# nianticlabs/implicit-depth

Measured on AMD Instinct MI355X. Metric: frames/sec (BDModel.forward hot path, 512x384, 64 planes, 8-frame tuple = 1 current + 7 source views; third-party backbones excluded), higher is better.
Workload: dtype f32

## Files before the change

implicit-depth_amd/_lib.py:

```python
from __future__ import annotations

import ctypes as C
import os

import torch

_HERE = os.path.dirname(os.path.abspath(__file__))
LIB_PATH = os.environ.get("IDH_LIB") or os.path.join(_HERE, "lib", "libidh.so")

_lib = None
MIN_ABI_VERSION = 111

f32p = C.c_void_p


class IdhError(RuntimeError):
    pass


class VolumeOpts(C.Structure):

    _fields_ = [("cur_batch_stride", C.c_int64), ("src_batch_stride", C.c_int64), ("planes", C.c_void_p),
                ("planes_batch_stride", C.c_int64), ("planes_plane_stride", C.c_int64), ("planes_pixel_stride", C.c_int32),
                ("kernel", C.c_int32), ("scratch", C.c_void_p), ("scratch_floats", C.c_int64), ("struct_size", C.c_int64)]

    def __init__(self, *a, **k):
        super().__init__(*a, **k)
        self.struct_size = C.sizeof(VolumeOpts)


CV_KERNEL_LANE, CV_KERNEL_QUAD, CV_KERNEL_WINDOW = 1, 2, 3


class EvalArgs(C.Structure):

    _fields_ = [("struct_size", C.c_int64), ("prediction", C.c_void_p), ("pred_kind", C.c_int32), ("sampling", C.c_int32),
                ("sigmoid_multiplier", C.c_float), ("surface_threshold", C.c_float), ("rendered_bphw", C.c_void_p), ("depth_b1hw", C.c_void_p),
                ("gt_b1HW", C.c_void_p), ("thresholds", C.c_void_p), ("bins", C.c_void_p), ("T", C.c_int32), ("n_bins", C.c_int32),
                ("tag_mask", C.c_int32), ("B", C.c_int32), ("P", C.c_int32), ("h", C.c_int32), ("w", C.c_int32), ("H", C.c_int32), ("W", C.c_int32)]
# ... 471 lines not shown
```

implicit-depth_amd/cost_volume.py:

```python
from __future__ import annotations

from typing import Optional

import torch
from torch import Tensor, nn

from . import _lib
from .geometry import BackprojectDepth, Project3D


def to_nhwc(x_nchw: Tensor) -> Tensor:
    _lib.require_cuda_f32(x_nchw)
    x = x_nchw.contiguous()
    *lead, C, H, W = x.shape
    n_img = 1
    for s in lead:
        n_img *= s
    out = torch.empty(*lead, H, W, C, device=x.device, dtype=torch.float32)
    if out.numel():
        _lib.check(_lib.lib().idh_nchw_to_nhwc_f32(_lib.ptr(x), _lib.ptr(out), n_img, C, H * W, _lib.stream_ptr()), "idh_nchw_to_nhwc_f32")
    return out


def to_nchw(x_nhwc: Tensor) -> Tensor:
# ... 2 lines not shown
    *lead, H, W, C = x.shape
    n_img = 1
    for s in lead:
        n_img *= s
    out = torch.empty(*lead, C, H, W, device=x.device, dtype=torch.float32)
    if out.numel():
        _lib.check(_lib.lib().idh_nhwc_to_nchw_f32(_lib.ptr(x), _lib.ptr(out), n_img, C, H * W, _lib.stream_ptr()), "idh_nhwc_to_nchw_f32")
    return out


def _is_device_scalar(v) -> bool:
    return torch.is_tensor(v) and v.is_cuda


def volume_opts(B, K, C, H, W, D, planes_bdhw: Optional[Tensor] = None, cur_batch_stride: int = 0, src_batch_stride: int = 0, kernel: int = 0,
                dot_scratch_device=None):
    n_scratch = int(_lib.lib().idh_cost_volume_dot_scratch_floats(B, K, C, H, W, D)) if dot_scratch_device is not None else 0
    if planes_bdhw is None and not cur_batch_stride and not src_batch_stride and not kernel and not n_scratch:
        return None, []
    o = _lib.VolumeOpts()
    o.cur_batch_stride, o.src_batch_stride, o.kernel = int(cur_batch_stride), int(src_batch_stride), int(kernel)
    keep = []
    if n_scratch:
        sc = torch.empty(n_scratch, device=dot_scratch_device, dtype=torch.float32)
        o.scratch, o.scratch_floats = sc.data_ptr(), n_scratch
        keep.append(sc)
    if planes_bdhw is not None:
        pl = planes_bdhw
        _lib.require_cuda_f32(pl)
        if pl.dim() != 4 or pl.shape[1] != D or pl.shape[0] not in (1, B) or tuple(pl.shape[2:]) not in ((H, W), (1, 1)):
            raise ValueError(f"depth_planes_bdhw has shape {tuple(pl.shape)}, expected ({B},{D},{H},{W})")
        const_over_image = tuple(pl.shape[2:]) == (1, 1) or (pl.stride(2) == 0 and pl.stride(3) == 0)
        if const_over_image:
            sb = pl.stride(0) if pl.shape[0] == B and B > 1 else 0
            o.planes, o.planes_batch_stride, o.planes_plane_stride, o.planes_pixel_stride = pl.data_ptr(), sb, pl.stride(1), 0
        else:
# ... 160 lines not shown
DEFAULT_MLP_MATH = "fp32"


class FeatureVolumeManager(CostVolumeManager):

    def __init__(self, matching_height, matching_width, num_depth_bins=64, mlp_channels=None, matching_dim_size=16, num_source_views=7):
        super().__init__(matching_height, matching_width, num_depth_bins)
        from .networks import MLP

        mlp_channels = list(mlp_channels) if mlp_channels is not None else [202, 128, 128, 1]
        mlp_channels[0] = matching_dim_size * (1 + num_source_views) + 10 * num_source_views + 4
        self.matching_dim_size = matching_dim_size
        self.num_source_views = num_source_views
        self.mlp = MLP(channel_list=mlp_channels, disable_final_activation=True)
        self.mlp_math: Optional[str] = None

    def _math(self) -> str:
        m = DEFAULT_MLP_MATH if self.__dict__.get("mlp_math") is None else self.mlp_math
        if m not in MLP_MATH_MODES:
            raise _lib.IdhError(f"unknown MLP math mode {m!r} (expected one of {MLP_MATH_MODES})")
        return m

    def _packed(self):
        lins = [self.mlp.net[0], self.mlp.net[2], self.mlp.net[4]]
        math = self._math()
        key = (math,) + tuple((p.data_ptr(), _lib.param_version(p)) for p in self.mlp.parameters())
        c = self.__dict__.get("_idh_fv")
        if c is not None and c[0] == key:
            return c[1]
        K, C = self.num_source_views, self.matching_dim_size
# ... 41 lines not shown
             planes_t=None, cur_batch_stride=0, src_batch_stride=0, scratch=None):
        B, K, C, H, W = dims
        if K != self.num_source_views:
            raise _lib.IdhError(f"FeatureVolumeManager was built for {self.num_source_views} source views, got {K} (the MLP input width is fixed)")
        pk = self._packed()
        L = _lib.lib()
        D = self.num_depth_bins
        sc = scratch if scratch is not None else {}
        key = ("fv", B, H, W, D, str(dev), torch.cuda.current_stream().cuda_stream)
        if sc.get("fv_key") != key:
            wsb = L.idh_feature_volume_workspace_bytes(B)
            sc.update(fv_key=key, fv_wsb=wsb, fv_ws=torch.empty(max(wsb // 4, 1), device=dev), fv_planes=torch.empty(D, device=dev))
        lowest = torch.empty(B, H, W, device=dev)
        mask = torch.empty(B, H, W, device=dev, dtype=torch.bool) if want_mask else None
        planes = sc["fv_planes"] if planes_t is None else None
        opts, keep = volume_opts(B, K, C, H, W, D, planes_t, cur_batch_stride, src_batch_stride)
        mats = [t if t.is_contiguous() else t.contiguous() for t in (src_Ks, src_extrinsics, src_poses, cur_invK)]
        _lib.check(
            L.idh_feature_volume_ex_fwd(cur_ptr, src_ptr, mats[0].data_ptr(), mats[1].data_ptr(), mats[2].data_ptr(), mats[3].data_ptr(),
                                        dmin, dmax, B, K, C, H, W, D,
                                        pk["w1v"].data_ptr(), pk["w1p"].data_ptr(), pk["pose"].data_ptr(), pk["b1"].data_ptr(), pk["w2"].data_ptr(),
                                        pk["vecs"].data_ptr(), vol_ptr, vol_cs, lowest.data_ptr(),
                                        _lib.ptr(mask), _lib.ptr(planes), sc["fv_ws"].data_ptr(), sc["fv_wsb"], int(pk["math"] == "f16x3"), opts,
                                        _lib.stream_ptr()),
            "idh_feature_volume_ex_fwd")
        del keep
        return lowest, planes, mask

    def build_cost_volume(self, cur_feats, src_feats, src_extrinsics, src_poses, src_Ks, cur_invK, min_depth, max_depth,
                          depth_planes_bdhw=None, return_mask=False, cur_feats_nhwc=None, src_feats_nhwc=None):
        B, K, C, H, W = self._check(cur_feats, src_feats)
# ... 28 lines not shown
```

implicit-depth_amd/csrc/feature_volume.hip:

```cpp
#include <stdlib.h>

#include "idh_common.h"
#include "split_f16.h"

namespace {

using namespace idh_f16;

constexpr int kC = 16;
constexpr int kHid = 128;
constexpr int kNS = 8;
constexpr int kMaxK = 8;

constexpr int kWsHom = 0, kWsT = 192, kWsInvK = 256, kWsBias = 272;
static_assert(kWsT == 12 * IDH_MAX_SOURCE_VIEWS && kWsInvK == kWsT + 4 * IDH_MAX_SOURCE_VIEWS && kWsBias + kHid <= 400, "workspace layout");
constexpr int kWsStrideReal = 400;

__device__ __forceinline__ float lrelu01(float x) {
#ifdef IDH_ABL_FV2_NOACT
    return x;
#endif
    return __builtin_elementwise_maximum(x, x * 0.01f);
}
__device__ __forceinline__ float lrelu01_sel(float x) { return x >= 0.f ? x : x * 0.01f; }

__device__ __forceinline__ float fv_depth_plane(int i, int D, float dmin, float dmax) {
    float ramp = 0.f;
    if (D > 1) {
        const float step = 1.0f / (float)(D - 1);
        ramp = (i < D / 2) ? step * (float)i : 1.0f - step * (float)(D - 1 - i);
    }
    return expf(logf(dmin) + logf(dmax / dmin) * ramp);
}

__global__ void fv_setup_k(const float *__restrict__ src_K, const float *__restrict__ src_E,
                           const float *__restrict__ src_poses, const float *__restrict__ cur_invK,
                           const float *__restrict__ w1_pose, const float *__restrict__ b1, int K,
                           float *__restrict__ ws) {
    const int b = blockIdx.x, t = threadIdx.x;
    float *o = ws + (size_t)b * kWsStrideReal;
    __shared__ float s_pd[3 * IDH_MAX_SOURCE_VIEWS];
    if (t < K) {
        const float *Km = src_K + (size_t)(b * K + t) * 16, *Em = src_E + (size_t)(b * K + t) * 16;
        const float *iK = cur_invK + (size_t)b * 16, *Pm = src_poses + (size_t)(b * K + t) * 16;
        float P[3][4];
        for (int i = 0; i < 3; ++i)
            for (int j = 0; j < 4; ++j) {
                float s = 0.f;
                for (int m = 0; m < 4; ++m) s = fmaf(Km[i * 4 + m], Em[m * 4 + j], s);
                P[i][j] = s;
            }
        float *h = o + kWsHom + 12 * t;
        for (int i = 0; i < 3; ++i) {
            for (int j = 0; j < 3; ++j) {
                float s = 0.f;
                for (int m = 0; m < 3; ++m) s = fmaf(P[i][m], iK[m * 4 + j], s);
                h[i * 3 + j] = s;
            }
            h[9 + i] = P[i][3];
        }
        o[kWsT + 4 * t + 0] = Pm[3]; o[kWsT + 4 * t + 1] = Pm[7]; o[kWsT + 4 * t + 2] = Pm[11]; o[kWsT + 4 * t + 3] = 0.f;
        const float tr = Pm[0] + Pm[5] + Pm[10];
        const float rm = sqrtf(2.f * (1.f - fminf(3.f, tr) / 3.f));
        const float tm = sqrtf(Pm[3] * Pm[3] + Pm[7] * Pm[7] + Pm[11] * Pm[11]);
        s_pd[t] = sqrtf(tm * tm + rm * rm);
        s_pd[K + t] = rm;
        s_pd[2 * K + t] = tm;
    }
    if (t < 9) o[kWsInvK + t] = cur_invK[(size_t)b * 16 + (t / 3) * 4 + (t % 3)];
    __syncthreads();
    if (t < kHid) {
        float s = b1[t];
        for (int j = 0; j < 3 * K; ++j) s = fmaf(w1_pose[(size_t)t * 3 * K + j], s_pd[j], s);
        o[kWsBias + t] = s;
    }
}

struct FvArgs {
    const float *cur;
    const float *src;
    const float *ws;
    const float *w1v;
    const float *w1p;
    const float *w2;
    const float *vecs;
    float *vol;
    unsigned char *mask;
    int vol_cs;
    int B, K, H, W, D;
    int tiles_per_img;
    int DP, G;
    int J, MB;
    float dmin, dmax;
    long long cur_bs, src_bs;
    const float *planes;
    long long planes_sb, planes_sd;
    int planes_sp;
};

__device__ __forceinline__ float fv_plane(const FvArgs &a, int b, int p, int d) {
    return a.planes ? a.planes[(size_t)b * a.planes_sb + (size_t)d * a.planes_sd + (size_t)p * a.planes_sp]
                    : fv_depth_plane(d, a.D, a.dmin, a.dmax);
}

template <int KT>
__global__ __launch_bounds__(512) void fv_mlp_k(const FvArgs a) {
    extern __shared__ __attribute__((aligned(16))) unsigned char smem_raw[];
    f32x4 *sW1 = reinterpret_cast<f32x4 *>(smem_raw);
    f32x4 *sW2 = sW1 + (a.K + 4) * kNS * 64;
    {
        const f32x4 *g1 = reinterpret_cast<const f32x4 *>(a.w1v);
        const f32x4 *g2 = reinterpret_cast<const f32x4 *>(a.w2);
        const int n1 = (a.K + 4) * kNS * 64, n2 = kNS * kNS * 64;
        for (int i = threadIdx.x; i < n1; i += 512) sW1[i] = g1[i];
        for (int i = threadIdx.x; i < n2; i += 512) sW2[i] = g2[i];
    }
    __syncthreads();
    const float *s_b2 = a.vecs, *s_w3 = a.vecs + kHid;
    const float b3 = a.vecs[2 * kHid];

    const int lane = threadIdx.x & 63;
// ... 285 lines not shown
                    const float qy = fmaf(hm[3], pxf, fmaf(hm[4], pyf, hm[5]));
                    const float qz = fmaf(hm[6], pxf, fmaf(hm[7], pyf, hm[8]));
                    const float cx = fmaf(depth, qx, hm[9]);
                    const float cy = fmaf(depth, qy, hm[10]);
                    const float cz = fmaf(depth, qz, hm[11]);
                    const float z = fmaxf(cz, 1e-5f);
                    float r = __builtin_amdgcn_rcpf(z);
                    r = r * fmaf(-z, r, 2.0f);
                    const float u = cx * r, v = cy * r;
                    any_inb |= (u > 2.f) & (u < Wf - 2.f) & (v > 2.f) & (v < Hf - 2.f);
                    any_front |= z > 0.f;
                }
                if (q == 0 && live) a.mask[(size_t)b * N + p] = (any_front && any_inb) ? 1 : 0;
            }
            P = Pn; cur = curn; wc = wcn;
        }
    }
}

template <int CB>
__global__ __launch_bounds__(512) void fv_mlp_gen_k(const FvArgs a) {
    extern __shared__ __attribute__((aligned(16))) unsigned char smem_raw[];
    f32x4 *sW2 = reinterpret_cast<f32x4 *>(smem_raw);
    {
        const f32x4 *g2 = reinterpret_cast<const f32x4 *>(a.w2);
        for (int i = threadIdx.x; i < kNS * kNS * 64; i += 512) sW2[i] = g2[i];
    }
    __syncthreads();
    const f32x4 *gW1 = reinterpret_cast<const f32x4 *>(a.w1v);
    const float *s_b2 = a.vecs, *s_w3 = a.vecs + kHid;
// ... 619 lines not shown
                               size_t workspace_bytes, void *stream, bool f16x3, const idh_volume_opts *opts) {
    const bool own_planes = opts && opts->planes;
    if (own_planes) { dmin = dmax = 1.f; planes_d = nullptr; }
    if (B < 0 || K <= 0 || H <= 0 || W <= 0 || D <= 0 || !(dmin > 0.f) || !(dmax > 0.f)) return IDH_EINVAL;
    const bool generic = C != kC || K > kMaxK;
    if ((long long)K * H * W * C * 4 >= (1ll << 31)) return IDH_EUNSUPPORTED;
    if ((C != kC && C != 2 * kC) || K > IDH_MAX_SOURCE_VIEWS || D > 4096 || (generic && f16x3)) return IDH_EUNSUPPORTED;
    if (B == 0) return IDH_OK;
    if (!cur_nhwc || !src_nhwc || !src_K_44 || !src_E_44 || !src_poses_44 || !cur_invK_44 || !w1_voxel_packed ||
        !w1_pixel_packed || !w1_pose_rowmajor || !b1 || !w2_packed || !vecs_b2_w3_b3 || !vol)
        return IDH_EINVAL;
    if (vol_nhwc_cs != 0 && vol_nhwc_cs < D) return IDH_EINVAL;
    if (!workspace || workspace_bytes < idh_feature_volume_workspace_bytes(B)) return IDH_EWORKSPACE;
    hipStream_t st = idh_stream(stream);
    float *ws = static_cast<float *>(workspace);
    hipLaunchKernelGGL(fv_setup_k, dim3(B), dim3(128), 0, st, src_K_44, src_E_44, src_poses_44, cur_invK_44,
                       w1_pose_rowmajor, b1, K, ws);
    IDH_CHECK_LAUNCH();

    FvArgs a{};
    a.cur = cur_nhwc; a.src = src_nhwc; a.ws = ws; a.w1v = static_cast<const float *>(w1_voxel_packed); a.w1p = w1_pixel_packed;
    a.w2 = static_cast<const float *>(w2_packed);
    a.vecs = vecs_b2_w3_b3; a.vol = vol; a.mask = mask_bhw; a.vol_cs = vol_nhwc_cs;
    a.B = B; a.K = K; a.H = H; a.W = W; a.D = D; a.dmin = dmin; a.dmax = dmax;
    const int N = H * W;
    a.cur_bs = (long long)N * C; a.src_bs = (long long)K * N * C;
    a.J = K <= kMaxK ? 2 : (K + 3) / 4;
    a.MB = 2 * a.J;
    if (opts) {
        if (opts->cur_batch_stride) a.cur_bs = opts->cur_batch_stride;
        if (opts->src_batch_stride) a.src_bs = opts->src_batch_stride;
        if (a.cur_bs < (long long)N * C || a.src_bs < (long long)K * N * C || (a.cur_bs & 3) || (a.src_bs & 3)) return IDH_EINVAL;
        if (opts->planes) {
            if (opts->planes_pixel_stride != 0 && opts->planes_pixel_stride != 1) return IDH_EINVAL;
            a.planes = opts->planes; a.planes_sb = opts->planes_batch_stride; a.planes_sd = opts->planes_plane_stride;
            a.planes_sp = opts->planes_pixel_stride;
        }
    }
    a.tiles_per_img = (N + 15) / 16;
    fv_plane_groups(B, H, W, D, &a.G, &a.DP);
    const long long pix_tasks = (long long)B * a.tiles_per_img;
    const long long ntasks = pix_tasks * a.G;
    int grid = (int)((ntasks + 7) / 8);
    if (grid > 256) grid = 256;
    static IdhDeviceOnce attr_set;
    if (attr_set.first()) {
        if (hipFuncSetAttribute(reinterpret_cast<const void *>(fv_mlp_k<0>), hipFuncAttributeMaxDynamicSharedMemorySize,
                                160 * 1024) != hipSuccess ||
            hipFuncSetAttribute(reinterpret_cast<const void *>(fv_mlp_gen_k<1>), hipFuncAttributeMaxDynamicSharedMemorySize, 64 * 1024) != hipSuccess ||
            hipFuncSetAttribute(reinterpret_cast<const void *>(fv_mlp_gen_k<2>), hipFuncAttributeMaxDynamicSharedMemorySize, 64 * 1024) != hipSuccess ||
            hipFuncSetAttribute(reinterpret_cast<const void *>(fv_mlp_k<7>), hipFuncAttributeMaxDynamicSharedMemorySize,
                                160 * 1024) != hipSuccess ||
            hipFuncSetAttribute(reinterpret_cast<const void *>(fv_mlp_k<8>), hipFuncAttributeMaxDynamicSharedMemorySize,
                                160 * 1024) != hipSuccess ||
            hipFuncSetAttribute(reinterpret_cast<const void *>(fv_mlp_f16_k<0>), hipFuncAttributeMaxDynamicSharedMemorySize,
                                160 * 1024) != hipSuccess ||
            hipFuncSetAttribute(reinterpret_cast<const void *>(fv_mlp_f16_k<7>), hipFuncAttributeMaxDynamicSharedMemorySize,
                                160 * 1024) != hipSuccess ||
            hipFuncSetAttribute(reinterpret_cast<const void *>(fv_mlp_f16_k<8>), hipFuncAttributeMaxDynamicSharedMemorySize,
                                160 * 1024) != hipSuccess)
            return IDH_ELAUNCH;
        attr_set.mark();
    }
    if (generic) {
        const size_t lds = (size_t)kNS * kNS * 64 * sizeof(f32x4);
        if (C == kC) hipLaunchKernelGGL(fv_mlp_gen_k<1>, dim3(grid), dim3(512), lds, st, a);
        else hipLaunchKernelGGL(fv_mlp_gen_k<2>, dim3(grid), dim3(512), lds, st, a);
    } else if (f16x3) {
        const int nb32 = (K + 5) / 2;
        const size_t lds = ((size_t)nb32 * kNS * 2 * 64 + 4 * kNS * 2 * 64) * 16;
        const float *sw1 = reinterpret_cast<const float *>(static_cast<const char *>(w1_voxel_packed) + (size_t)nb32 * kNS * 2 * 64 * 16);
        const float *sw2 = reinterpret_cast<const float *>(static_cast<const char *>(w2_packed) + (size_t)4 * kNS * 2 * 64 * 16);
        if (K == 7) hipLaunchKernelGGL(fv_mlp_f16_k<7>, dim3(grid), dim3(512), lds, st, a, sw1, sw2);
        else if (K == 8) hipLaunchKernelGGL(fv_mlp_f16_k<8>, dim3(grid), dim3(512), lds, st, a, sw1, sw2);
        else hipLaunchKernelGGL(fv_mlp_f16_k<0>, dim3(grid), dim3(512), lds, st, a, sw1, sw2);
    } else {
        const size_t lds = ((size_t)(K + 4) * kNS * 64 + kNS * kNS * 64) * sizeof(f32x4);
        if (K == 7) hipLaunchKernelGGL(fv_mlp_k<7>, dim3(grid), dim3(512), lds, st, a);
        else if (K == 8) hipLaunchKernelGGL(fv_mlp_k<8>, dim3(grid), dim3(512), lds, st, a);
        else hipLaunchKernelGGL(fv_mlp_k<0>, dim3(grid), dim3(512), lds, st, a);
    }
    IDH_CHECK_LAUNCH();
    if (lowest_bhw) {
        int g2 = idh_cdiv((long long)B * N, vol_nhwc_cs > 0 ? 16 : 256);
        if (g2 > 8192) g2 = 8192;
        hipLaunchKernelGGL(argmax_planes_k, dim3(g2), dim3(256), 0, st, vol, vol_nhwc_cs, B, N, D, dmin, dmax, lowest_bhw,
                           planes_d, a.planes, a.planes_sb, a.planes_sd, a.planes_sp);
        IDH_CHECK_LAUNCH();
    }
    return IDH_OK;
}
```

include/idh.h:

```cpp
#ifndef IDH_H_
#define IDH_H_

#include <stddef.h>
#include <stdint.h>

#ifdef __cplusplus
extern "C" {
#endif
#if defined(__GNUC__) || defined(__clang__)
#pragma GCC visibility push(default)
#endif

#define IDH_OK 0
#define IDH_EINVAL (-1)
#define IDH_EUNSUPPORTED (-2)
#define IDH_ELAUNCH (-3)
#define IDH_EWORKSPACE (-4)

#define IDH_MAX_SOURCE_VIEWS 16

#define IDH_ACT_NONE 0
#define IDH_ACT_LRELU 1
#define IDH_ACT_ELU 2

// ... 2 lines not shown

int idh_nchw_to_nhwc_f32(const float *src_nchw, float *dst_nhwc, int n_img, int C, int HW, void *stream);
int idh_nhwc_to_nchw_f32(const float *src_nhwc, float *dst_nchw, int n_img, int C, int HW, void *stream);

typedef struct idh_volume_opts {
    int64_t cur_batch_stride;
    int64_t src_batch_stride;
    const float *planes;
    int64_t planes_batch_stride;
    int64_t planes_plane_stride;
    int32_t planes_pixel_stride;
    int32_t kernel;
    float *scratch;
    int64_t scratch_floats;
    int64_t struct_size;
} idh_volume_opts;

size_t idh_sizeof_volume_opts(void);

#define IDH_CV_KERNEL_LANE 1
#define IDH_CV_KERNEL_QUAD 2
#define IDH_CV_KERNEL_WINDOW 3

int idh_cost_volume_dot_fwd(const float *cur_nhwc, const float *src_nhwc, const float *src_K_44,
                            const float *src_E_44, const float *cur_invK_44, float dmin, float dmax,
                            int B, int K, int C, int H, int W, int D, float *cost, int cost_nhwc_cs,
                            float *lowest_bhw, float *planes_d, void *stream);
int idh_cost_volume_dot_ex_fwd(const float *cur_nhwc, const float *src_nhwc, const float *src_K_44,
                               const float *src_E_44, const float *cur_invK_44, float dmin, float dmax,
                               int B, int K, int C, int H, int W, int D, float *cost, int cost_nhwc_cs,
// ... 177 lines not shown
```

Before: 690.3.

## Skip MLP work for source views that project outside the image

Adds a sampled visibility estimate in the setup kernel that measures what fraction of source-view projections fall outside the image. A new skip kernel variant computes an active-view mask per plane and runs the layer-1 accumulation only for views with in-bounds taps. It is used when enough views are empty, with both kernels launched and each exiting early depending on the device-side estimate. This aims to cut wasted bilinear gathers and MFMA work on out-of-frustum views, at the cost of an extra launch, divergent loops, and reliance on those views contributing zero features.

```diff
diff --git a/implicit-depth_amd/_lib.py b/implicit-depth_amd/_lib.py
--- a/implicit-depth_amd/_lib.py
+++ b/implicit-depth_amd/_lib.py
@@ -22,7 +22,8 @@
 
     _fields_ = [("cur_batch_stride", C.c_int64), ("src_batch_stride", C.c_int64), ("planes", C.c_void_p),
                 ("planes_batch_stride", C.c_int64), ("planes_plane_stride", C.c_int64), ("planes_pixel_stride", C.c_int32),
-                ("kernel", C.c_int32), ("scratch", C.c_void_p), ("scratch_floats", C.c_int64), ("struct_size", C.c_int64)]
+                ("kernel", C.c_int32), ("scratch", C.c_void_p), ("scratch_floats", C.c_int64), ("struct_size", C.c_int64),
+                ("fv_keep_empty_views", C.c_int32), ("reserved0", C.c_int32)]
 
     def __init__(self, *a, **k):
         super().__init__(*a, **k)
diff --git a/implicit-depth_amd/cost_volume.py b/implicit-depth_amd/cost_volume.py
--- a/implicit-depth_amd/cost_volume.py
+++ b/implicit-depth_amd/cost_volume.py
@@ -40,12 +40,13 @@
 
 
 def volume_opts(B, K, C, H, W, D, planes_bdhw: Optional[Tensor] = None, cur_batch_stride: int = 0, src_batch_stride: int = 0, kernel: int = 0,
-                dot_scratch_device=None):
+                dot_scratch_device=None, fv_keep_empty_views: int = 0):
     n_scratch = int(_lib.lib().idh_cost_volume_dot_scratch_floats(B, K, C, H, W, D)) if dot_scratch_device is not None else 0
-    if planes_bdhw is None and not cur_batch_stride and not src_batch_stride and not kernel and not n_scratch:
+    if planes_bdhw is None and not cur_batch_stride and not src_batch_stride and not kernel and not n_scratch and not fv_keep_empty_views:
         return None, []
     o = _lib.VolumeOpts()
     o.cur_batch_stride, o.src_batch_stride, o.kernel = int(cur_batch_stride), int(src_batch_stride), int(kernel)
+    o.fv_keep_empty_views = int(fv_keep_empty_views)
     keep = []
     if n_scratch:
         sc = torch.empty(n_scratch, device=dot_scratch_device, dtype=torch.float32)
@@ -236,6 +237,7 @@
         self.num_source_views = num_source_views
         self.mlp = MLP(channel_list=mlp_channels, disable_final_activation=True)
         self.mlp_math: Optional[str] = None
+        self.skip_empty_views = True
 
     def _math(self) -> str:
         m = DEFAULT_MLP_MATH if self.__dict__.get("mlp_math") is None else self.mlp_math
@@ -307,7 +309,8 @@
         lowest = torch.empty(B, H, W, device=dev)
         mask = torch.empty(B, H, W, device=dev, dtype=torch.bool) if want_mask else None
         planes = sc["fv_planes"] if planes_t is None else None
-        opts, keep = volume_opts(B, K, C, H, W, D, planes_t, cur_batch_stride, src_batch_stride)
+        opts, keep = volume_opts(B, K, C, H, W, D, planes_t, cur_batch_stride, src_batch_stride,
+                                 fv_keep_empty_views={True: 0, False: 1, "always": 2}[self.__dict__.get("skip_empty_views", True)])
         mats = [t if t.is_contiguous() else t.contiguous() for t in (src_Ks, src_extrinsics, src_poses, cur_invK)]
         _lib.check(
             L.idh_feature_volume_ex_fwd(cur_ptr, src_ptr, mats[0].data_ptr(), mats[1].data_ptr(), mats[2].data_ptr(), mats[3].data_ptr(),
diff --git a/implicit-depth_amd/csrc/feature_volume.hip b/implicit-depth_amd/csrc/feature_volume.hip
--- a/implicit-depth_amd/csrc/feature_volume.hip
+++ b/implicit-depth_amd/csrc/feature_volume.hip
@@ -31,49 +31,6 @@
         ramp = (i < D / 2) ? step * (float)i : 1.0f - step * (float)(D - 1 - i);
     }
     return expf(logf(dmin) + logf(dmax / dmin) * ramp);
-}
-
-__global__ void fv_setup_k(const float *__restrict__ src_K, const float *__restrict__ src_E,
-                           const float *__restrict__ src_poses, const float *__restrict__ cur_invK,
-                           const float *__restrict__ w1_pose, const float *__restrict__ b1, int K,
-                           float *__restrict__ ws) {
-    const int b = blockIdx.x, t = threadIdx.x;
-    float *o = ws + (size_t)b * kWsStrideReal;
-    __shared__ float s_pd[3 * IDH_MAX_SOURCE_VIEWS];
-    if (t < K) {
-        const float *Km = src_K + (size_t)(b * K + t) * 16, *Em = src_E + (size_t)(b * K + t) * 16;
-        const float *iK = cur_invK + (size_t)b * 16, *Pm = src_poses + (size_t)(b * K + t) * 16;
-        float P[3][4];
-        for (int i = 0; i < 3; ++i)
-            for (int j = 0; j < 4; ++j) {
-                float s = 0.f;
-                for (int m = 0; m < 4; ++m) s = fmaf(Km[i * 4 + m], Em[m * 4 + j], s);
-                P[i][j] = s;
-            }
-        float *h = o + kWsHom + 12 * t;
-        for (int i = 0; i < 3; ++i) {
-            for (int j = 0; j < 3; ++j) {
-                float s = 0.f;
-                for (int m = 0; m < 3; ++m) s = fmaf(P[i][m], iK[m * 4 + j], s);
-                h[i * 3 + j] = s;
-            }
-            h[9 + i] = P[i][3];
-        }
-        o[kWsT + 4 * t + 0] = Pm[3]; o[kWsT + 4 * t + 1] = Pm[7]; o[kWsT + 4 * t + 2] = Pm[11]; o[kWsT + 4 * t + 3] = 0.f;
-        const float tr = Pm[0] + Pm[5] + Pm[10];
-        const float rm = sqrtf(2.f * (1.f - fminf(3.f, tr) / 3.f));
-        const float tm = sqrtf(Pm[3] * Pm[3] + Pm[7] * Pm[7] + Pm[11] * Pm[11]);
-        s_pd[t] = sqrtf(tm * tm + rm * rm);
-        s_pd[K + t] = rm;
-        s_pd[2 * K + t] = tm;
-    }
-    if (t < 9) o[kWsInvK + t] = cur_invK[(size_t)b * 16 + (t / 3) * 4 + (t % 3)];
-    __syncthreads();
-    if (t < kHid) {
-        float s = b1[t];
-        for (int j = 0; j < 3 * K; ++j) s = fmaf(w1_pose[(size_t)t * 3 * K + j], s_pd[j], s);
-        o[kWsBias + t] = s;
-    }
 }
 
 struct FvArgs {
@@ -96,6 +53,7 @@
     const float *planes;
     long long planes_sb, planes_sd;
     int planes_sp;
+    int select;
 };
 
 __device__ __forceinline__ float fv_plane(const FvArgs &a, int b, int p, int d) {
@@ -103,8 +61,89 @@
                     : fv_depth_plane(d, a.D, a.dmin, a.dmax);
 }
 
+constexpr int kWsOutside = 265;
+constexpr float kSkipMinOutside = 0.25f;
+__device__ __forceinline__ bool fv_selected(const FvArgs &a, bool skipping_kernel) {
+    if (a.select == 0) return true;
+    float s = 0.f;
+    for (int b = threadIdx.x & 63; b < a.B; b += 64) s += a.ws[(size_t)b * kWsStrideReal + kWsOutside];
+#pragma unroll
+    for (int o = 32; o > 0; o >>= 1) s += __shfl_xor(s, o, 64);
+    return (s >= kSkipMinOutside * (float)a.B) == skipping_kernel;
+}
+
+__global__ void fv_setup_k(const float *__restrict__ src_K, const float *__restrict__ src_E,
+                           const float *__restrict__ src_poses, const float *__restrict__ cur_invK,
+                           const float *__restrict__ w1_pose, const float *__restrict__ b1, int K,
+                           float *__restrict__ ws, const FvArgs a) {
+    const int b = blockIdx.x, t = threadIdx.x;
+    float *o = ws + (size_t)b * kWsStrideReal;
+    __shared__ float s_pd[3 * IDH_MAX_SOURCE_VIEWS];
+    if (t < K) {
+        const float *Km = src_K + (size_t)(b * K + t) * 16, *Em = src_E + (size_t)(b * K + t) * 16;
+        const float *iK = cur_invK + (size_t)b * 16, *Pm = src_poses + (size_t)(b * K + t) * 16;
+        float P[3][4];
+        for (int i = 0; i < 3; ++i)
+            for (int j = 0; j < 4; ++j) {
+                float s = 0.f;
+                for (int m = 0; m < 4; ++m) s = fmaf(Km[i * 4 + m], Em[m * 4 + j], s);
+                P[i][j] = s;
+            }
+        float *h = o + kWsHom + 12 * t;
+        for (int i = 0; i < 3; ++i) {
+            for (int j = 0; j < 3; ++j) {
+                float s = 0.f;
+                for (int m = 0; m < 3; ++m) s = fmaf(P[i][m], iK[m * 4 + j], s);
+                h[i * 3 + j] = s;
+            }
+            h[9 + i] = P[i][3];
+        }
+        o[kWsT + 4 * t + 0] = Pm[3]; o[kWsT + 4 * t + 1] = Pm[7]; o[kWsT + 4 * t + 2] = Pm[11]; o[kWsT + 4 * t + 3] = 0.f;
+        const float tr = Pm[0] + Pm[5] + Pm[10];
+        const float rm = sqrtf(2.f * (1.f - fminf(3.f, tr) / 3.f));
+        const float tm = sqrtf(Pm[3] * Pm[3] + Pm[7] * Pm[7] + Pm[11] * Pm[11]);
+        s_pd[t] = sqrtf(tm * tm + rm * rm);
+        s_pd[K + t] = rm;
+        s_pd[2 * K + t] = tm;
+    }
+    if (t < 9) o[kWsInvK + t] = cur_invK[(size_t)b * 16 + (t / 3) * 4 + (t % 3)];
+    __syncthreads();
+    if (t < kHid) {
+        float s = b1[t];
+        for (int j = 0; j < 3 * K; ++j) s = fmaf(w1_pose[(size_t)t * 3 * K + j], s_pd[j], s);
+        o[kWsBias + t] = s;
+    }
+    if (a.select == 0) return;
+    __shared__ int s_out;
+    if (t == 0) s_out = 0;
+    __syncthreads();
+    const int px = ((2 * (t & 15) + 1) * a.W) >> 5, py = ((2 * (t >> 4) + 1) * a.H) >> 4;
+    const float pxf = (float)px + 0.5f, pyf = (float)py + 0.5f, Wf = (float)a.W, Hf = (float)a.H;
+    int n_out = 0;
+    const int nd = min(a.D, 8);
+    float dj[8];
+#pragma unroll
+    for (int j = 0; j < 8; ++j) dj[j] = fv_plane(a, b, py * a.W + px, ((2 * min(j, nd - 1) + 1) * a.D) / (2 * nd));
+    for (int k = 0; k < K; ++k) {
+        const float *hm = o + kWsHom + 12 * k;
+        const float qx = fmaf(hm[0], pxf, fmaf(hm[1], pyf, hm[2])), hx = hm[9];
+        const float qy = fmaf(hm[3], pxf, fmaf(hm[4], pyf, hm[5])), hy = hm[10];
+        const float qz = fmaf(hm[6], pxf, fmaf(hm[7], pyf, hm[8])), hz = hm[11];
+#pragma unroll
+        for (int j = 0; j < 8; ++j) {
+            const float z = fmaxf(fmaf(dj[j], qz, hz), 1e-5f);
+            const float sx = fmaf(dj[j], qx, hx) / z - 0.5f, sy = fmaf(dj[j], qy, hy) / z - 0.5f;
+            n_out += (j < nd) && !(sx > -1.f && sx < Wf && sy > -1.f && sy < Hf);
+        }
+    }
+    atomicAdd(&s_out, n_out);
+    __syncthreads();
+    if (t == 0) o[kWsOutside] = (float)s_out / (float)(128 * K * nd);
+}
+
 template <int KT>
 __global__ __launch_bounds__(512) void fv_mlp_k(const FvArgs a) {
+    if (!fv_selected(a, false)) return;
     extern __shared__ __attribute__((aligned(16))) unsigned char smem_raw[];
     f32x4 *sW1 = reinterpret_cast<f32x4 *>(smem_raw);
     f32x4 *sW2 = sW1 + (a.K + 4) * kNS * 64;
@@ -420,6 +459,433 @@
                 if (q == 0 && live) a.mask[(size_t)b * N + p] = (any_front && any_inb) ? 1 : 0;
             }
             P = Pn; cur = curn; wc = wcn;
+        }
+    }
+}
+
+template <int KT>
+__global__ __launch_bounds__(512) void fv_mlp_skip_k(const FvArgs a) {
+    if (!fv_selected(a, true)) return;
+    extern __shared__ __attribute__((aligned(16))) unsigned char smem_raw[];
+    f32x4 *sW1 = reinterpret_cast<f32x4 *>(smem_raw);
+    f32x4 *sW2 = sW1 + (a.K + 4) * kNS * 64;
+    {
+        const f32x4 *g1 = reinterpret_cast<const f32x4 *>(a.w1v);
+        const f32x4 *g2 = reinterpret_cast<const f32x4 *>(a.w2);
+        const int n1 = (a.K + 4) * kNS * 64, n2 = kNS * kNS * 64;
+        for (int i = threadIdx.x; i < n1; i += 512) sW1[i] = g1[i];
+        for (int i = threadIdx.x; i < n2; i += 512) sW2[i] = g2[i];
+    }
+    __syncthreads();
+    const float *s_b2 = a.vecs, *s_w3 = a.vecs + kHid;
+    const float b3 = a.vecs[2 * kHid];
+
+    const int lane = threadIdx.x & 63;
+    const int wave = __builtin_amdgcn_readfirstlane(threadIdx.x >> 6);
+    const int ln = lane & 15, q = lane >> 4;
+    const int N = a.H * a.W;
+    const int K = KT > 0 ? KT : a.K;
+    const float Wf = (float)a.W, Hf = (float)a.H;
+    const long long ntasks = (long long)a.B * a.tiles_per_img * a.G;
+
+    for (long long task = (long long)idh_xcd_remap(blockIdx.x, gridDim.x) * 8 + wave; task < ntasks; task += (long long)gridDim.x * 8) {
+        const int g = __builtin_amdgcn_readfirstlane((int)(task % a.G));
+        const int tile = __builtin_amdgcn_readfirstlane((int)((task / a.G) % a.tiles_per_img));
+        const int b = __builtin_amdgcn_readfirstlane((int)(task / ((long long)a.G * a.tiles_per_img)));
+        const int p_raw = tile * 16 + ln;
+        const bool live = p_raw < N;
+        const int p = live ? p_raw : N - 1;
+        const int py = p / a.W, px = p - py * a.W;
+        const float pxf = (float)px + 0.5f, pyf = (float)py + 0.5f;
+        const float *pb = a.ws + (size_t)b * kWsStrideReal;
+
+        const f32x4 cur4 = *reinterpret_cast<const f32x4 *>(a.cur + (size_t)b * a.cur_bs + (size_t)p * kC + 4 * q);
+        const float *iK = pb + kWsInvK;
+        const float rx = fmaf(iK[0], pxf, fmaf(iK[1], pyf, iK[2]));
+        const float ry = fmaf(iK[3], pxf, fmaf(iK[4], pyf, iK[5]));
+        const float rz = fmaf(iK[6], pxf, fmaf(iK[7], pyf, iK[8]));
+
+        f32x4 pre[kNS];
+#pragma unroll
+        for (int i = 0; i < kNS; ++i) pre[i] = *reinterpret_cast<const f32x4 *>(pb + kWsBias + 16 * i + 4 * q);
+        const int d0 = g * a.DP, d1 = min(a.D, d0 + a.DP);
+        if (d0 >= d1) continue;
+        const float rn = fmaxf(sqrtf(rx * rx + ry * ry + rz * rz), 1e-12f);
+        const float crx = rx / rn, cry = ry / rn, crz = rz / rn;
+        {
+            const f32x4 rayB = (q == 0) ? (f32x4){crx, cry, crz, 0.f} : (f32x4){0.f, 0.f, 0.f, 0.f};
+            const __amdgpu_buffer_rsrc_t rsP = __builtin_amdgcn_make_buffer_rsrc(const_cast<float *>(a.w1p), 0, 2 * kNS * 64 * 16, 0x00020000);
+#pragma unroll
+            for (int i = 0; i < kNS; ++i) {
+                const f32x4 A0 = __builtin_bit_cast(f32x4, __builtin_amdgcn_raw_buffer_load_b128(rsP, 16 * lane, (0 * kNS + i) * 1024, 0));
+                const f32x4 A1 = __builtin_bit_cast(f32x4, __builtin_amdgcn_raw_buffer_load_b128(rsP, 16 * lane, (1 * kNS + i) * 1024, 0));
+#pragma unroll
+                for (int kk = 0; kk < 4; ++kk) pre[i] = __builtin_amdgcn_mfma_f32_16x16x4f32(A0[kk], cur4[kk], pre[i], 0, 0, 0);
+#pragma unroll
+                for (int kk = 0; kk < 4; ++kk) pre[i] = __builtin_amdgcn_mfma_f32_16x16x4f32(A1[kk], rayB[kk], pre[i], 0, 0, 0);
+            }
+        }
+
+        const int ov[2] = {min(q, K - 1), min(q + 4, K - 1)};
+        float oq[2][3], oh[2][3];
+#pragma unroll
+        for (int jv = 0; jv < 2; ++jv) {
+            const float *hm = pb + kWsHom + 12 * ov[jv];
+            oq[jv][0] = fmaf(hm[0], pxf, fmaf(hm[1], pyf, hm[2]));
+            oq[jv][1] = fmaf(hm[3], pxf, fmaf(hm[4], pyf, hm[5]));
+            oq[jv][2] = fmaf(hm[6], pxf, fmaf(hm[7], pyf, hm[8]));
+            oh[jv][0] = hm[9]; oh[jv][1] = hm[10]; oh[jv][2] = hm[11];
+        }
+        const __amdgpu_buffer_rsrc_t rsS = __builtin_amdgcn_make_buffer_rsrc(const_cast<float *>(a.src + (size_t)b * a.src_bs), 0, K * N * kC * 4, 0x00020000);
+        const int bp0 = 4 * ln;
+
+        f32x4 ob = (f32x4){0.f, 0.f, 0.f, 0.f};
+        const bool vec_ok = ((d0 & 3) == 0) && ((a.vol_cs & 3) == 0) && ((reinterpret_cast<uintptr_t>(a.vol) & 15) == 0);
+        struct Own { int pk; float w00, w01, w10, w11, z; };
+        struct Pro { Own own[2]; float depth, m3, m4, m5, m6, m10, m11, m12, m13; };
+        struct Tap { f32x4 t00, t01, t10, t11; };
+        struct Wts { float w00, w01, w10, w11; };
+        float oc[2][3];
+#pragma unroll
+        for (int jv = 0; jv < 2; ++jv) {
+            const float *t = pb + kWsT + 4 * ov[jv];
+            oc[jv][0] = t[0]; oc[jv][1] = t[1]; oc[jv][2] = t[2];
+        }
+        auto prologue = [&](int d) {
+            Pro P;
+            const float depth = fv_plane(a, b, p, d);
+            P.depth = depth;
+#pragma unroll
+            for (int jv = 0; jv < 2; ++jv) {
+#ifdef IDH_ABL_FV2_NOPRO
+                P.own[jv].pk = p; P.own[jv].w00 = P.own[jv].w01 = P.own[jv].w10 = P.own[jv].w11 = depth; P.own[jv].z = depth;
+                continue;
+#endif
+                const float cx = fmaf(depth, oq[jv][0], oh[jv][0]);
+                const float cy = fmaf(depth, oq[jv][1], oh[jv][1]);
+                const float cz = fmaf(depth, oq[jv][2], oh[jv][2]);
+                const float z = fmaxf(cz, 1e-5f);
+                float r = __builtin_amdgcn_rcpf(z);
+                r = r * fmaf(-z, r, 2.0f);
+                const float su = cx * r, sv = cy * r;
+                const float sx = fminf(fmaxf(su - 0.5f, -1.0f), Wf);
+                const float sy = fminf(fmaxf(sv - 0.5f, -1.0f), Hf);
+                const float x0f = floorf(sx), y0f = floorf(sy);
+                const float fx = sx - x0f, fy = sy - y0f;
+                const int x0 = (int)x0f, y0 = (int)y0f;
+                const float wx0 = (x0 >= 0 && x0 < a.W) ? 1.0f - fx : 0.f;
+                const float wx1 = (x0 + 1 < a.W) ? fx : 0.f;
+                const float wy0 = (y0 >= 0 && y0 < a.H) ? 1.0f - fy : 0.f;
+                const float wy1 = (y0 + 1 < a.H) ? fy : 0.f;
+                const int xa0 = min(max(x0, 0), a.W - 1), xa1 = min(x0 + 1, a.W - 1);
+                const int ya0 = min(max(y0, 0), a.H - 1), ya1 = min(y0 + 1, a.H - 1);
+                P.own[jv].pk = (ya0 * a.W + xa0) | ((xa1 - xa0) << 30) | ((ya1 - ya0) << 31);
+                P.own[jv].w00 = wx0 * wy0; P.own[jv].w01 = wx1 * wy0; P.own[jv].w10 = wx0 * wy1; P.own[jv].w11 = wx1 * wy1;
+                P.own[jv].z = z;
+            }
+            const float Xx = depth * rx, Xy = depth * ry, Xz = depth * rz;
+            auto ray = [&](int jv, float &ang, float &e0, float &e1, float &e2) {
+                const float ax = Xx - oc[jv][0], ay = Xy - oc[jv][1], az = Xz - oc[jv][2];
+                const float n2 = fmaf(az, az, fmaf(ay, ay, ax * ax));
+                float in = __builtin_amdgcn_rsqf(fmaxf(n2, 1e-24f));
+                in = in * fmaf(-0.5f * n2 * in, in, 1.5f);
+                e0 = ax * in; e1 = ay * in; e2 = az * in;
+                ang = fmaf(crz, e2, fmaf(cry, e1, crx * e0));
+            };
+#ifdef IDH_ABL_FV2_NORAY
+            P.m3 = P.m4 = P.m5 = P.m6 = P.m10 = P.m11 = P.m12 = P.m13 = depth;
+            return P;
+#endif
+            ray(0, P.m3, P.m4, P.m5, P.m6);
+            ray(1, P.m10, P.m11, P.m12, P.m13);
+            return P;
+        };
+        auto issue = [&](const Pro &P, int k) {
+            const int pk = __builtin_amdgcn_ds_bpermute(bp0 + 64 * (k & 3), P.own[k >> 2].pk);
+            const int o00 = ((pk & 0x3fffffff) << 6) + 16 * q;
+            const int o01 = o00 + (((pk >> 30) & 1) << 6);
+            const int ystep = (int)((unsigned)pk >> 31) * (a.W * 64);
+            Tap t;
+#ifdef IDH_ABL_FV2_NOTAPS
+            t.t00 = t.t01 = t.t10 = t.t11 = (f32x4){1.f + (float)o00, 2.f + (float)o01, 3.f + (float)ystep, 4.f};
+            return t;
+#endif
+            const int so = __builtin_amdgcn_readfirstlane(k * N * (kC * 4));
+            t.t00 = __builtin_bit_cast(f32x4, __builtin_amdgcn_raw_buffer_load_b128(rsS, o00, so, 0));
+            t.t01 = __builtin_bit_cast(f32x4, __builtin_amdgcn_raw_buffer_load_b128(rsS, o01, so, 0));
+            t.t10 = __builtin_bit_cast(f32x4, __builtin_amdgcn_raw_buffer_load_b128(rsS, o00 + ystep, so, 0));
+            t.t11 = __builtin_bit_cast(f32x4, __builtin_amdgcn_raw_buffer_load_b128(rsS, o01 + ystep, so, 0));
+            return t;
+        };
+        auto weights = [&](const Pro &P, int k) {
+            const Own &o = P.own[k >> 2];
+            auto bperm = [&](float v) -> float { return __builtin_bit_cast(float, __builtin_amdgcn_ds_bpermute(bp0 + 64 * (k & 3), __builtin_bit_cast(int, v))); };
+            Wts w;
+            w.w00 = bperm(o.w00); w.w01 = bperm(o.w01); w.w10 = bperm(o.w10); w.w11 = bperm(o.w11);
+            return w;
+        };
+        const unsigned all_views = (1u << K) - 1u;
+        auto active = [&](const Pro &P) -> unsigned {
+            auto nz = [](const Own &o) {
+                return (__builtin_bit_cast(int, o.w00) | __builtin_bit_cast(int, o.w01) | __builtin_bit_cast(int, o.w10) | __builtin_bit_cast(int, o.w11)) != 0;
+            };
+            const unsigned long long b0 = __ballot(nz(P.own[0])), b1 = __ballot(nz(P.own[1]));
+            unsigned m = 0;
+#pragma unroll
+            for (int j = 0; j < 4; ++j) {
+                m |= ((unsigned)(b0 >> (16 * j)) & 0xffffu) ? (1u << j) : 0u;
+                m |= ((unsigned)(b1 >> (16 * j)) & 0xffffu) ? (16u << j) : 0u;
+            }
+            return (unsigned)__builtin_amdgcn_readfirstlane((int)(m & all_views));
+        };
+        auto issue_rt = [&](const Pro &P, int k, bool none) {
+            const int own_pk = (k & 4) ? P.own[1].pk : P.own[0].pk;
+            const int pk = __builtin_amdgcn_ds_bpermute(bp0 + 64 * (k & 3), own_pk);
+            const unsigned o00 = max((unsigned)(((pk & 0x3fffffff) << 6) + 16 * q), none ? 0x7ffffff0u : 0u);
+            const unsigned o01 = o00 + (unsigned)(((pk >> 30) & 1) << 6);
+            const unsigned ystep = ((unsigned)pk >> 31) * (unsigned)(a.W * 64);
+            Tap t;
+#ifdef IDH_ABL_FV2_NOTAPS
+            t.t00 = t.t01 = t.t10 = t.t11 = (f32x4){1.f + (float)o00, 2.f + (float)o01, 3.f + (float)ystep, 4.f};
+            return t;
+#endif
+            const int so = __builtin_amdgcn_readfirstlane(k * N * (kC * 4));
+            t.t00 = __builtin_bit_cast(f32x4, __builtin_amdgcn_raw_buffer_load_b128(rsS, (int)o00, so, 0));
+            t.t01 = __builtin_bit_cast(f32x4, __builtin_amdgcn_raw_buffer_load_b128(rsS, (int)o01, so, 0));
+            t.t10 = __builtin_bit_cast(f32x4, __builtin_amdgcn_raw_buffer_load_b128(rsS, (int)(o00 + ystep), so, 0));
+            t.t11 = __builtin_bit_cast(f32x4, __builtin_amdgcn_raw_buffer_load_b128(rsS, (int)(o01 + ystep), so, 0));
+            return t;
+        };
+        auto weights_rt = [&](const Pro &P, int k) {
+            const bool hi = (k & 4) != 0;
+            auto bperm = [&](float v) -> float { return __builtin_bit_cast(float, __builtin_amdgcn_ds_bpermute(bp0 + 64 * (k & 3), __builtin_bit_cast(int, v))); };
+            Wts w;
+            w.w00 = bperm(hi ? P.own[1].w00 : P.own[0].w00); w.w01 = bperm(hi ? P.own[1].w01 : P.own[0].w01);
+            w.w10 = bperm(hi ? P.own[1].w10 : P.own[0].w10); w.w11 = bperm(hi ? P.own[1].w11 : P.own[0].w11);
+            return w;
+        };
+        auto first_view = [&](unsigned act) { return act ? __builtin_ctz(act) : 0; };
+        Pro P = prologue(d0);
+        unsigned act = active(P);
+        Tap cur = issue_rt(P, first_view(act), act == 0);
+        Wts wc = weights_rt(P, first_view(act));
+#pragma unroll 1
+        for (int d = d0; d < d1; ++d) {
+            const float depth = P.depth;
+            f32x4 acc1[kNS], acc2[kNS];
+            float m2 = 0.f, m9 = 0.f;
+            const float m1 = q < K ? P.own[0].z : 0.f;
+            float m8 = q + 4 < K ? P.own[1].z : 0.f;
+            __builtin_amdgcn_s_setprio(2);
+            constexpr int KU = KT > 0 ? KT : kMaxK;
+            auto layer2_chunk = [&](int c) {
+#pragma unroll
+                for (int i = 0; i < kNS; ++i) {
+#ifdef IDH_ABL_FV2_NOLDSA
+                    const f32x4 A = (f32x4){1.f, 2.f, 3.f, 4.f} * (float)(i + 1);
+#else
+                    const f32x4 A = sW2[(c * kNS + i) * 64 + lane];
+#endif
+#pragma unroll
+                    for (int kk = 0; kk < 4; ++kk) acc2[i] = __builtin_amdgcn_mfma_f32_16x16x4f32(A[kk], acc1[c][kk], acc2[i], 0, 0, 0);
+                }
+            };
+            auto layer1_tail = [&]() {
+                const float m3 = P.m3, m4 = P.m4, m5 = P.m5, m6 = P.m6, m10 = P.m10, m11 = P.m11, m12 = P.m12, m13 = P.m13;
+                const bool depth_in_q3 = K < 8;
+                if (depth_in_q3 && q == 3) m8 = depth;
+                const f32x4 mb[4] = {(f32x4){m1, m2, m3, m4}, (f32x4){m5, m6, m8, m9}, (f32x4){m10, m11, m12, m13}, (f32x4){depth, 0.f, 0.f, 0.f}};
+#pragma unroll
+                for (int c = 0; c < 3; ++c) {
+#pragma unroll
+                    for (int i = 0; i < kNS; ++i) {
+                        const f32x4 A = sW1[((K + c) * kNS + i) * 64 + lane];
+#pragma unroll
+                        for (int kk = 0; kk < 4; ++kk) acc1[i] = __builtin_amdgcn_mfma_f32_16x16x4f32(A[kk], mb[c][kk], acc1[i], 0, 0, 0);
+                    }
+                }
+                if (!depth_in_q3) {
+#pragma unroll
+                    for (int i = 0; i < kNS; ++i) {
+                        const float A0 = reinterpret_cast<const float *>(&sW1[((K + 3) * kNS + i) * 64 + lane])[0];
+                        acc1[i] = __builtin_amdgcn_mfma_f32_16x16x4f32(A0, mb[3][0], acc1[i], 0, 0, 0);
+                    }
+                }
+#pragma unroll
+                for (int r = 0; r < 4; ++r) acc1[0][r] = lrelu01(acc1[0][r]);
+#pragma unroll
+                for (int i = 0; i < kNS; ++i) acc2[i] = *reinterpret_cast<const f32x4 *>(s_b2 + 16 * i + 4 * q);
+                __builtin_amdgcn_s_setprio(0);
+                layer2_chunk(0);
+            };
+            auto view_rt = [&](int k, const Tap &cur, const Wts &wc) {
+                f32x4 wv;
+#ifdef IDH_ABL_FV2_NOBLEND
+                wv = cur.t00 + cur.t11;
+                float part = wc.w00 + wc.w11 + cur.t01[0] + cur.t10[0];
+#else
+#pragma unroll
+                for (int e = 0; e < 4; ++e)
+                    wv[e] = fmaf(wc.w11, cur.t11[e], fmaf(wc.w10, cur.t10[e], fmaf(wc.w01, cur.t01[e], wc.w00 * cur.t00[e])));
+                float part = wv[0] * cur4[0];
+                part = fmaf(wv[1], cur4[1], part); part = fmaf(wv[2], cur4[2], part); part = fmaf(wv[3], cur4[3], part);
+                part += __shfl_xor(part, 16, 64);
+                part += __shfl_xor(part, 32, 64);
+#endif
+                m2 = (k == q) ? part : m2;
+                m9 = (k == q + 4) ? part : m9;
+#pragma unroll
+                for (int i = 0; i < kNS; ++i) {
+#ifdef IDH_ABL_FV2_NOLDSA
+                    const f32x4 A = (f32x4){1.f, 2.f, 3.f, 4.f} * (float)(i + 1);
+#else
+                    const f32x4 A = sW1[(k * kNS + i) * 64 + lane];
+#endif
+#pragma unroll
+                    for (int kk = 0; kk < 4; ++kk) acc1[i] = __builtin_amdgcn_mfma_f32_16x16x4f32(A[kk], wv[kk], acc1[i], 0, 0, 0);
+                }
+            };
+            if (act == all_views) {
+#pragma unroll
+                for (int i = 0; i < kNS; ++i) acc1[i] = pre[i];
+#pragma unroll
+                for (int k = 0; k < KU; ++k) {
+                    if (KT == 0 && k >= K) break;
+                    const int kn = (KT > 0) ? (k + 1 < KT ? k + 1 : k) : k + 1;
+                    Tap nxt = cur;
+                    Wts wn = wc;
+                    if (kn != k && kn < KU) { nxt = issue(P, kn); wn = weights(P, kn); }
+                    f32x4 wv;
+#ifdef IDH_ABL_FV2_NOBLEND
+                    wv = cur.t00 + cur.t11;
+                    float part = wc.w00 + wc.w11 + cur.t01[0] + cur.t10[0];
+#else
+#pragma unroll
+                    for (int e = 0; e < 4; ++e)
+                        wv[e] = fmaf(wc.w11, cur.t11[e], fmaf(wc.w10, cur.t10[e], fmaf(wc.w01, cur.t01[e], wc.w00 * cur.t00[e])));
+                    float part = wv[0] * cur4[0];
+                    part = fmaf(wv[1], cur4[1], part); part = fmaf(wv[2], cur4[2], part); part = fmaf(wv[3], cur4[3], part);
+                    part += __shfl_xor(part, 16, 64);
+                    part += __shfl_xor(part, 32, 64);
+#endif
+                    const float dotv = part;
+                    const bool s0 = (k == q), s1 = (k == q + 4);
+                    m2 = s0 ? dotv : m2;
+                    m9 = s1 ? dotv : m9;
+#pragma unroll
+                    for (int i = 0; i < kNS; ++i) {
+#ifdef IDH_ABL_FV2_NOLDSA
+                        const f32x4 A = (f32x4){1.f, 2.f, 3.f, 4.f} * (float)(i + 1);
+#else
+                        const f32x4 A = sW1[(k * kNS + i) * 64 + lane];
+#endif
+#pragma unroll
+                        for (int kk = 0; kk < 4; ++kk) acc1[i] = __builtin_amdgcn_mfma_f32_16x16x4f32(A[kk], wv[kk], acc1[i], 0, 0, 0);
+                    }
+                    if constexpr (KT > 0) {
+#pragma unroll
+                        for (int r = 0; r < 16; ++r) {
+                            __builtin_amdgcn_sched_group_barrier(0x008, 2, 0);
+#ifndef IDH_ABL_FV_VALU_PER_GROUP
+#define IDH_ABL_FV_VALU_PER_GROUP 3
+#endif
+                            __builtin_amdgcn_sched_group_barrier(0x002, IDH_ABL_FV_VALU_PER_GROUP, 0);
+                        }
+                    }
+                    cur = nxt;
+                    wc = wn;
+                }
+                layer1_tail();
+            } else {
+#pragma unroll
+                for (int i = 0; i < kNS; ++i) acc1[i] = pre[i];
+                if (act != 0) {
+                    int k = __builtin_ctz(act);
+                    unsigned rem = act & (act - 1u);
+#pragma unroll 1
+                    while (rem != 0) {
+                        const int kn = __builtin_ctz(rem);
+                        rem &= rem - 1u;
+                        const Tap nxt = issue_rt(P, kn, false);
+                        const Wts wn = weights_rt(P, kn);
+                        view_rt(k, cur, wc);
+                        cur = nxt;
+                        wc = wn;
+                        k = kn;
+                    }
+                    view_rt(k, cur, wc);
+                }
+                layer1_tail();
+            }
+#pragma unroll
+            for (int i = 1; i < kNS; ++i) {
+#pragma unroll
+                for (int r = 0; r < 4; ++r) acc1[i][r] = lrelu01(acc1[i][r]);
+            }
+            Pro Pn;
+            Tap curn;
+            Wts wcn;
+            unsigned actn = 0;
+            auto next_plane = [&]() {
+                Pn = prologue(min(d + 1, d1 - 1));
+                actn = active(Pn);
+                curn = issue_rt(Pn, first_view(actn), actn == 0);
+                wcn = weights_rt(Pn, first_view(actn));
+            };
+            if constexpr (KT > 0) next_plane();
+            else __builtin_amdgcn_sched_barrier(0);
+#pragma unroll
+            for (int c = 1; c < kNS; ++c) {
+                layer2_chunk(c);
+                if (KT == 0 && c == 1) next_plane();
+                if constexpr (KT == 0) __builtin_amdgcn_sched_barrier(0);
+            }
+            float s = 0.f;
+#ifdef IDH_ABL_FV2_NOL3
+#pragma unroll
+            for (int i = 0; i < kNS; ++i) s += acc2[i][0];
+#else
+#pragma unroll
+            for (int i = 0; i < kNS; ++i) {
+                const f32x4 w3 = *reinterpret_cast<const f32x4 *>(s_w3 + 16 * i + 4 * q);
+#pragma unroll
+                for (int r = 0; r < 4; ++r) s = fmaf(w3[r], lrelu01(acc2[i][r]), s);
+            }
+            s += __shfl_xor(s, 16, 64);
+            s += __shfl_xor(s, 32, 64);
+#endif
+            const float val = s + b3;
+            if (a.vol_cs > 0) {
+                const int e = (d - d0) & 3;
+                ob[0] = e == 0 ? val : ob[0]; ob[1] = e == 1 ? val : ob[1]; ob[2] = e == 2 ? val : ob[2]; ob[3] = e == 3 ? val : ob[3];
+                if (q == 0 && live && (e == 3 || d == d1 - 1)) {
+                    float *o = a.vol + ((size_t)b * N + p) * a.vol_cs + (d - e);
+                    if (e == 3 && vec_ok) *reinterpret_cast<f32x4 *>(o) = ob;
+                    else { o[0] = ob[0]; if (e >= 1) o[1] = ob[1]; if (e >= 2) o[2] = ob[2]; if (e >= 3) o[3] = ob[3]; }
+                }
+            } else if (q == 0 && live) {
+                a.vol[((size_t)b * a.D + d) * N + p] = val;
+            }
+            if (a.mask != nullptr && d == a.D - 1) {
+                bool any_inb = false, any_front = false;
+                for (int k = 0; k < K; ++k) {
+                    const float *hm = pb + kWsHom + 12 * k;
+                    const float qx = fmaf(hm[0], pxf, fmaf(hm[1], pyf, hm[2]));
+                    const float qy = fmaf(hm[3], pxf, fmaf(hm[4], pyf, hm[5]));
+                    const float qz = fmaf(hm[6], pxf, fmaf(hm[7], pyf, hm[8]));
+                    const float cx = fmaf(depth, qx, hm[9]);
+                    const float cy = fmaf(depth, qy, hm[10]);
+                    const float cz = fmaf(depth, qz, hm[11]);
+                    const float z = fmaxf(cz, 1e-5f);
+                    float r = __builtin_amdgcn_rcpf(z);
+                    r = r * fmaf(-z, r, 2.0f);
+                    const float u = cx * r, v = cy * r;
+                    any_inb |= (u > 2.f) & (u < Wf - 2.f) & (v > 2.f) & (v < Hf - 2.f);
+                    any_front |= z > 0.f;
+                }
+                if (q == 0 && live) a.mask[(size_t)b * N + p] = (any_front && any_inb) ? 1 : 0;
+            }
+            P = Pn; cur = curn; wc = wcn; act = actn;
         }
     }
 }
@@ -1069,11 +1535,9 @@
     if (!workspace || workspace_bytes < idh_feature_volume_workspace_bytes(B)) return IDH_EWORKSPACE;
     hipStream_t st = idh_stream(stream);
     float *ws = static_cast<float *>(workspace);
-    hipLaunchKernelGGL(fv_setup_k, dim3(B), dim3(128), 0, st, src_K_44, src_E_44, src_poses_44, cur_invK_44,
-                       w1_pose_rowmajor, b1, K, ws);
-    IDH_CHECK_LAUNCH();
 
     FvArgs a{};
+    int views_mode = 0;
     a.cur = cur_nhwc; a.src = src_nhwc; a.ws = ws; a.w1v = static_cast<const float *>(w1_voxel_packed); a.w1p = w1_pixel_packed;
     a.w2 = static_cast<const float *>(w2_packed);
     a.vecs = vecs_b2_w3_b3; a.vol = vol; a.mask = mask_bhw; a.vol_cs = vol_nhwc_cs;
@@ -1091,8 +1555,14 @@
             a.planes = opts->planes; a.planes_sb = opts->planes_batch_stride; a.planes_sd = opts->planes_plane_stride;
             a.planes_sp = opts->planes_pixel_stride;
         }
+        if (opts->struct_size >= (int64_t)(offsetof(idh_volume_opts, fv_keep_empty_views) + sizeof(int32_t))) views_mode = opts->fv_keep_empty_views;
+        if (views_mode < 0 || views_mode > 2) return IDH_EINVAL;
     }
     a.tiles_per_img = (N + 15) / 16;
+    a.select = (!generic && !f16x3 && views_mode == 0) ? 1 : 0;
+    hipLaunchKernelGGL(fv_setup_k, dim3(B), dim3(128), 0, st, src_K_44, src_E_44, src_poses_44, cur_invK_44,
+                       w1_pose_rowmajor, b1, K, ws, a);
+    IDH_CHECK_LAUNCH();
     fv_plane_groups(B, H, W, D, &a.G, &a.DP);
     const long long pix_tasks = (long long)B * a.tiles_per_img;
     const long long ntasks = pix_tasks * a.G;
@@ -1106,6 +1576,9 @@
             hipFuncSetAttribute(reinterpret_cast<const void *>(fv_mlp_gen_k<2>), hipFuncAttributeMaxDynamicSharedMemorySize, 64 * 1024) != hipSuccess ||
             hipFuncSetAttribute(reinterpret_cast<const void *>(fv_mlp_k<7>), hipFuncAttributeMaxDynamicSharedMemorySize,
                                 160 * 1024) != hipSuccess ||
+            hipFuncSetAttribute(reinterpret_cast<const void *>(fv_mlp_skip_k<0>), hipFuncAttributeMaxDynamicSharedMemorySize, 160 * 1024) != hipSuccess ||
+            hipFuncSetAttribute(reinterpret_cast<const void *>(fv_mlp_skip_k<7>), hipFuncAttributeMaxDynamicSharedMemorySize, 160 * 1024) != hipSuccess ||
+            hipFuncSetAttribute(reinterpret_cast<const void *>(fv_mlp_skip_k<8>), hipFuncAttributeMaxDynamicSharedMemorySize, 160 * 1024) != hipSuccess ||
             hipFuncSetAttribute(reinterpret_cast<const void *>(fv_mlp_k<8>), hipFuncAttributeMaxDynamicSharedMemorySize,
                                 160 * 1024) != hipSuccess ||
             hipFuncSetAttribute(reinterpret_cast<const void *>(fv_mlp_f16_k<0>), hipFuncAttributeMaxDynamicSharedMemorySize,
@@ -1131,9 +1604,17 @@
         else hipLaunchKernelGGL(fv_mlp_f16_k<0>, dim3(grid), dim3(512), lds, st, a, sw1, sw2);
     } else {
         const size_t lds = ((size_t)(K + 4) * kNS * 64 + kNS * kNS * 64) * sizeof(f32x4);
-        if (K == 7) hipLaunchKernelGGL(fv_mlp_k<7>, dim3(grid), dim3(512), lds, st, a);
-        else if (K == 8) hipLaunchKernelGGL(fv_mlp_k<8>, dim3(grid), dim3(512), lds, st, a);
-        else hipLaunchKernelGGL(fv_mlp_k<0>, dim3(grid), dim3(512), lds, st, a);
+        if (views_mode != 2) {
+            if (K == 7) hipLaunchKernelGGL(fv_mlp_k<7>, dim3(grid), dim3(512), lds, st, a);
+            else if (K == 8) hipLaunchKernelGGL(fv_mlp_k<8>, dim3(grid), dim3(512), lds, st, a);
+            else hipLaunchKernelGGL(fv_mlp_k<0>, dim3(grid), dim3(512), lds, st, a);
+            IDH_CHECK_LAUNCH();
+        }
+        if (views_mode != 1) {
+            if (K == 7) hipLaunchKernelGGL(fv_mlp_skip_k<7>, dim3(grid), dim3(512), lds, st, a);
+            else if (K == 8) hipLaunchKernelGGL(fv_mlp_skip_k<8>, dim3(grid), dim3(512), lds, st, a);
+            else hipLaunchKernelGGL(fv_mlp_skip_k<0>, dim3(grid), dim3(512), lds, st, a);
+        }
     }
     IDH_CHECK_LAUNCH();
     if (lowest_bhw) {
diff --git a/include/idh.h b/include/idh.h
--- a/include/idh.h
+++ b/include/idh.h
@@ -40,6 +40,8 @@
     float *scratch;
     int64_t scratch_floats;
     int64_t struct_size;
+    int32_t fv_keep_empty_views;
+    int32_t reserved0;
 } idh_volume_opts;
 
 size_t idh_sizeof_volume_opts(void);
```

New measurement: 710.5, median of 6. +2.9%, better.
